# slinderman/pyglm

Hardware: AMD Instinct MI355X
Metric: Gibbs sweeps/sec (full resample_model) (higher is better)
Workload: dtype f64 (likelihood Gram: exact integer arithmetic on 13 i8 residue planes, CRT back to f64)

## Files before the change

### include/pyglm_hip.h

```cpp
#ifndef PYGLM_HIP_H
#define PYGLM_HIP_H
#include <stddef.h>
#include <stdint.h>
#ifdef __cplusplus
extern "C" {
#endif

#define PGL_ABI_VERSION 11

int pgl_abi_version(void);
const char* pgl_last_error(void);

int pgl_philox_words(uint64_t seed, uint32_t purpose, uint32_t j, uint64_t elem0, uint64_t stream, uint32_t* out, size_t n, void* hip_stream);

int pgl_pg_draw(const double* b, const double* z, double* out, size_t len, uint64_t seed, uint64_t stream, uint64_t elem0, void* hip_stream);

int pgl_design_matrix(const double* S, long lds, const double* basis, double* X, long ldx, double* Xt, long ldxt, int T, int N, int B, int R,
                      int clip, void* hip_stream);
int pgl_transpose(const double* src, long ld_src, double* dst, long ld_dst, int rows, int cols, void* hip_stream);

int pgl_activation(const double* Xt, long ldxt, const double* Wt, long ldw, double* Psi, long ldpsi, int T, int Dk, int nloc, void* hip_stream);

int pgl_pg_loglik(double* Psi, long ldpsi, const double* bias, const double* Y, long ldy, double* Omega, long ldo, double* Kappa, long ldk,
                  double* llpart, double* ll_out, int accumulate, int T, int nloc, int obs, double xi, uint64_t seed, uint64_t sweep,
// ... 111 lines not shown
    int obs; double xi;
    int visit_order;
    int planes, i8_group;
    const pgl_dataset_t* datasets; int ndatasets;
    int* a; double* W; double* b;
    const double* rho;
    const double* Jw; const double* hw; const int* label;
    const double* Jb; const double* hb;
    const double* c0;
    const int* perm; const double* u; const double* z;
    const double* inv_eta; const double* G0;
    double* ll;
    int* status;
    double* logodds;
    double* Wt; double* bias; double* border; int* skip; double* c0_dense;
    double* Jbuf; double* Mtab; double* Ac;
    double* hc; double* Tinv; double* G; double* Lws;
    double* Ut; double* Wt_ws;
    int* d_idx; double* d_sign; int* d_cnt; int* batch_k;
    int* act; int* na;
    void* i8_PB; void* i8_R; double* i8_stat;
    int i8_slice;
    void* i8_PAs;
    void* i8_Rx;
    double* i8_norm;
    int nrun;
    int nfirst;
    int all_deterministic;
    int init_rows_bound;
    int active_rows_bound;
    int flip_single_pass;
    pgl_stage_times_t* times;
    const double* obs_param;
} pgl_sweep_t;

int pgl_sweep_dims(int N, int B, int nloc, int* Dp, int* ldn, int* ldj);
int pgl_row_stats(const int* a, const double* W, double* out, int N, int B, int nloc, int n0, void* hip_stream);
int pgl_sweep(const pgl_sweep_t* s, uint64_t seed, uint64_t sweep, void* hip_stream);
int pgl_sweep_gram(const pgl_sweep_t* s, int first, int count, void* hip_stream);
int pgl_get_state(const pgl_sweep_t* s, int* a_host, double* W_host, double* b_host, double* ll_host, int* status_host, void* hip_stream);
const char* pgl_stage_name(int i);
int pgl_stage_times_collect(pgl_stage_times_t* t);

int pgl_summary_fold(const double* Psi, long ldn, const double* bias, const double* Y, double* llpart, double* ll_out, int accumulate, int T,
                     int nloc, int obs, double xi, const double* param, const double* hooks, long ldh, const double* inv_eta, double* rate_mean,
                     double* rate_M2, const int* link, int link0, const double* link_par, double link_par0, double* l_mean, double* l_M2,
                     double* lse_m, double* lse_s, int k, void* hip_stream);
int pgl_summary_state(const int* a, const double* Wt, long ldw, const double* bias, double* edge, double* w_mean, double* w_M2, double* b_mean,
                      double* b_M2, int N, int B, int nloc, int k, void* hip_stream);
int pgl_summary_colsum(const double* V, long ldv, int T, int nloc, double* part, double* out, int accumulate, void* hip_stream);

size_t pgl_generate_work_bytes(int N, int B);
int pgl_generate(const double* Wm, const double* bias, const double* basis, int N, int B, int L, int obs, double noise_scale, const double* U,
                 double* ring, double* Y, long t0, int Tc, void* work, int* status, void* hip_stream);

#define PGL_SIM_BINOMIAL_MAX_N 64
size_t pgl_simulate_work_bytes(int N, int B, int R);
int pgl_simulate(const double* Wm, const double* bias, const double* basis, int N, int B, int L, const int* kind, const double* par, int R,
                 long rep0, unsigned long long seed, double* ring, double* Y, long ldr, double* sum, double* sumsq, long t0, int Tc,
                 void* work, int* status, void* hip_stream);

#define PGL_LAG_MAX 256
#define PGL_LAG_I8 0
#define PGL_LAG_F64 1
size_t pgl_lagged_work_bytes(int N, int K, int R, int rows);
int pgl_lagged_products(const double* Y, long ldy, long strideY, int rows, int prev, int N, int K, int R, double* S, long strideS, int accumulate,
// ... 24 lines not shown
```

### pyglm_amd/_lib.py

```python
import ctypes
import os

_HERE = os.path.dirname(os.path.abspath(__file__))
LIB_PATH = os.path.join(_HERE, "lib", "libpyglm_hip.so")

c_p, c_l, c_i, c_d, c_u64, c_u32, c_sz = (ctypes.c_void_p, ctypes.c_long, ctypes.c_int, ctypes.c_double,
                                          ctypes.c_uint64, ctypes.c_uint32, ctypes.c_size_t)


class FlipState(ctypes.Structure):
    _fields_ = [("M", c_p), ("ldj", c_l), ("strideM", c_l), ("nb", c_i), ("N", c_i), ("B", c_i),
                ("perm", c_p), ("u", c_p), ("rho", c_p), ("c0", c_p), ("a", c_p), ("skip", c_p),
                ("d_idx", c_p), ("d_sign", c_p), ("d_cnt", c_p), ("batch_k", c_p), ("G", c_p), ("Lws", c_p),
                ("Ut", c_p), ("Wt", c_p), ("ldu", c_l), ("status", c_p), ("visit_order", c_i), ("logodds", c_p)]


class CholState(ctypes.Structure):
    _fields_ = [("J", c_p), ("ldj", c_l), ("strideJ", c_l), ("a", c_p), ("act", c_p), ("ldact", c_l), ("na", c_p),
                ("Ac", c_p), ("ldc", c_l), ("strideC", c_l), ("hc", c_p), ("Tinv", c_p), ("z", c_p), ("ldz", c_l),
                ("W", c_p), ("b", c_p), ("nb", c_i), ("N", c_i), ("B", c_i), ("status", c_p)]


class Dataset(ctypes.Structure):
    _fields_ = [("T", c_i), ("Tp", c_i), ("X", c_p), ("Xt", c_p), ("Y", c_p), ("Psi", c_p), ("OK", c_p), ("llpart", c_p), ("elem0", c_u64),
                ("int8", c_i), ("planes", c_i), ("sA", c_p), ("PA", c_p), ("omega_override", c_p), ("xmax", c_p),
                ("hooks", c_p)]


NSTAGES = 16


class StageTimes(ctypes.Structure):
    _fields_ = [("ms", c_d * NSTAGES), ("work", c_d * NSTAGES), ("calls", c_i * NSTAGES), ("pending", c_p), ("mask", c_u32)]


class Sweep(ctypes.Structure):
    _fields_ = [("N", c_i), ("B", c_i), ("n0", c_i), ("nloc", c_i), ("nb", c_i), ("obs", c_i), ("xi", c_d), ("visit_order", c_i),
                ("planes", c_i), ("i8_group", c_i), ("datasets", ctypes.POINTER(Dataset)), ("ndatasets", c_i),
                ("a", c_p), ("W", c_p), ("b", c_p), ("rho", c_p), ("Jw", c_p), ("hw", c_p), ("label", c_p), ("Jb", c_p), ("hb", c_p), ("c0", c_p),
                ("perm", c_p), ("u", c_p), ("z", c_p), ("inv_eta", c_p), ("G0", c_p), ("ll", c_p), ("status", c_p), ("logodds", c_p),
                ("Wt", c_p), ("bias", c_p), ("border", c_p), ("skip", c_p), ("c0_dense", c_p),
                ("Jbuf", c_p), ("Mtab", c_p), ("Ac", c_p), ("hc", c_p), ("Tinv", c_p), ("G", c_p), ("Lws", c_p), ("Ut", c_p), ("Wt_ws", c_p),
                ("d_idx", c_p), ("d_sign", c_p), ("d_cnt", c_p), ("batch_k", c_p), ("act", c_p), ("na", c_p),
                ("i8_PB", c_p), ("i8_R", c_p), ("i8_stat", c_p), ("i8_slice", c_i), ("i8_PAs", c_p), ("i8_Rx", c_p), ("i8_norm", c_p), ("nrun", c_i), ("nfirst", c_i),
                ("all_deterministic", c_i), ("init_rows_bound", c_i), ("active_rows_bound", c_i), ("flip_single_pass", c_i),
                ("times", ctypes.POINTER(StageTimes)), ("obs_param", c_p)]


SIGNATURES = {
    "pgl_abi_version": [],
    "pgl_last_error": [],
    "pgl_philox_words": [c_u64, c_u32, c_u32, c_u64, c_u64, c_p, c_sz, c_p],
    "pgl_pg_draw": [c_p, c_p, c_p, c_sz, c_u64, c_u64, c_u64, c_p],
    "pgl_design_matrix": [c_p, c_l, c_p, c_p, c_l, c_p, c_l, c_i, c_i, c_i, c_i, c_i, c_p],
    "pgl_transpose": [c_p, c_l, c_p, c_l, c_i, c_i, c_p],
    "pgl_activation": [c_p, c_l, c_p, c_l, c_p, c_l, c_i, c_i, c_i, c_p],
    "pgl_pg_loglik": [c_p, c_l, c_p, c_p, c_l, c_p, c_l, c_p, c_l, c_p, c_p, c_i, c_i, c_i, c_i, c_d, c_u64, c_u64, c_u64, c_u64, c_p],
    "pgl_pg_loglik_partials": [c_i],
    "pgl_pg_loglik_ex": [c_p, c_l, c_p, c_p, c_l, c_p, c_l, c_p, c_l, c_p, c_p, c_i, c_i, c_i, c_i, c_d, c_p, c_p, c_l, c_u64, c_u64, c_u64, c_u64, c_p],
    "pgl_gaussian_stats": [c_p, c_l, c_p, c_p, c_l, c_p, c_p, c_l, c_p, c_l, c_p, c_p, c_i, c_i, c_i, c_p],
    "pgl_scaled_gram": [c_p, c_l, c_p, c_p, c_l, c_l, c_i, c_i, c_p],
    "pgl_weighted_gram": [c_p, c_l, c_i, c_p, c_l, c_i, c_i, c_i, c_p, c_l, c_l, c_i, c_p],
    "pgl_i8_plane_bytes": [c_i, c_i],
    "pgl_i8_residue_bytes": [c_i],
    "pgl_i8_max_planes": [],
    "pgl_i8_padded_rows": [c_i],
    "pgl_i8_min_planes": [c_i],
    "pgl_i8_norm_bits": [c_i, c_i],
    "pgl_i8_norm_limit": [c_i, c_i],
    "pgl_i8_colstats": [c_p, c_l, c_p, c_l, c_i, c_i, c_i, c_p, c_p, c_p],
    "pgl_i8_scales": [c_p, c_p, c_l, c_i, c_i, c_p, c_p],
    "pgl_i8_planes": [c_p, c_l, c_p, c_l, c_p, c_p, c_i, c_i, c_i, c_i, c_l, c_p],
    "pgl_i8_planes_t": [c_p, c_l, c_p, c_l, c_p, c_p, c_i, c_i, c_i, c_i, c_l, c_p],
    "pgl_i8_gram": [c_p, c_p, c_p, c_i, c_i, c_i, c_i, c_p],
    "pgl_i8_gram_slice": [c_p, c_i, c_i, c_p, c_p, c_i, c_i, c_i, c_i, c_i, c_i, c_p],
    "pgl_i8_crt": [c_p, c_p, c_p, c_p, c_l, c_l, c_i, c_i, c_i, c_i, c_i, c_p],
    "pgl_contract_tn": [c_p, c_l, c_i, c_p, c_l, c_i, c_p, c_l, c_i, c_i, c_i, c_d, c_d, c_p],
    "pgl_contract_tn_batched": [c_p, c_l, c_l, c_i, c_p, c_l, c_l, c_i, c_p, c_l, c_l, c_i, c_i, c_i, c_i, c_p, c_d, c_d, c_i, c_i, c_p],
    "pgl_assemble_posterior": [c_p, c_l, c_l, c_p, c_p, c_l, c_p, c_p, c_p, c_p, c_p, c_i, c_i, c_i, c_p],
# ... 87 lines not shown
```

### pyglm_amd/csrc/pgl_common.h

```cpp
#pragma once
#include <hip/hip_runtime.h>
#include <stdint.h>
#include <stddef.h>
#include <atomic>
#include "../../include/pyglm_hip.h"

#define PGL_OK 0
#define PGL_ERR_ARG 1
#define PGL_ERR_HIP 2

void pgl_set_error(const char* fmt, ...);

#ifdef PGL_AB
#include <cstdlib>
inline int pgl_ab_int(const char* name, int dflt) { const char* e = getenv(name); return e ? atoi(e) : dflt; }
#else
constexpr int pgl_ab_int(const char*, int dflt) { return dflt; }
#endif

constexpr int PGL_MAX_DEVICES = 32;
int pgl_device();
int pgl_device_cus(int dev);
struct PglPerDevice {
    std::atomic<uint32_t> mask{0};
// ... 10 lines not shown
            pgl_set_error("%s:%d: argument check failed: %s", __FILE__, __LINE__, #cond); \
            return PGL_ERR_ARG;                                                          \
        }                                                                                \
    } while (0)

#define PGL_CHECK_LAUNCH()                                                                         \
    do {                                                                                           \
        hipError_t e_ = hipGetLastError();                                                         \
        if (e_ != hipSuccess) {                                                                    \
            pgl_set_error("%s:%d: kernel launch failed: %s", __FILE__, __LINE__, hipGetErrorString(e_)); \
            return PGL_ERR_HIP;                                                                    \
        }                                                                                          \
    } while (0)

typedef double d4_t __attribute__((ext_vector_type(4)));
typedef double d2_t __attribute__((ext_vector_type(2)));

struct PglGemmArgs {
    const double* A; long lda; long strideA;
    const double* B; long ldb; long strideB;
    double* C; long ldc; long strideC;
    const double* W; long ldw;
    int M, N, K;
    int a_cols, b_cols;
    int nbatch;
    int nz_total;
    double alpha, beta;
    int tri;
    const int* batch_k;
    int* sched;
    const int* batch_dim; int dim_off;
    int dim_mode;
    const int* batch_row_off;
    int pipe;
    int ksplit; long ks_rows; double* Cpart; long part_stride_z, part_stride_s;
};
enum PglGemmKind { PGL_GEMM_GRAM2 = 0, PGL_GEMM_PLAIN = 1, PGL_GEMM_TRI1 = 2, PGL_GEMM_SQUARES = 3 };
int pgl_launch_gemm(PglGemmKind kind, const PglGemmArgs& a, hipStream_t st);
int pgl_gram_split(const double* X, long ldx, int x_cols, const double* W, long ldw, int Tp, int D, int nz, double* J, long ldj, long strideJ, int accumulate,
                   long ks_rows, double* part, long part_stride_z, hipStream_t st);
bool pgl_update_supported(const PglGemmArgs& a);
int pgl_launch_update(const PglGemmArgs& a, hipStream_t st);
int pgl_launch_update_rows(const PglGemmArgs& a, int row0, int nrows, hipStream_t st);
int* pgl_sched_slot(hipStream_t st);

int pgl_k_philox_words(uint64_t, uint32_t, uint32_t, uint64_t, uint64_t, uint32_t*, size_t, hipStream_t);
int pgl_k_pg_draw(const double*, const double*, double*, size_t, uint64_t, uint64_t, uint64_t, hipStream_t);
int pgl_k_row_stats(const int* a, const double* W, double* out, int N, int B, int nloc, int n0, hipStream_t st);
int pgl_k_colsum_partials(const double* part, int nblk, int ncol, double* out, int accumulate, hipStream_t st);
int pgl_k_summary_state(const int* a, const double* Wt, long ldw, const double* bias, double* edge, double* wmean, double* wM2, double* bmean,
                        double* bM2, int N, int B, int nloc, int k, hipStream_t st);
int pgl_k_summary_colsum(const double* V, long ldv, int T, int nloc, double* part, double* out, int accumulate, hipStream_t st);
int pgl_k_scaled_gram(const double*, long, const double*, double*, long, long, int, int, hipStream_t);
int pgl_k_basis_conv(const double*, long, const double*, double*, long, double*, long, int, int, int, int, int, hipStream_t);
int pgl_k_transpose(const double*, long, double*, long, int, int, hipStream_t);
int pgl_k_assemble_post(double*, long, long, const double*, const double*, long, const double*, const double*, const int*, const double*,
                        const double*, int, int, int, hipStream_t);
size_t pgl_k_i8_plane_bytes(int, int);
size_t pgl_k_i8_residue_bytes(int);
int pgl_k_i8_max_planes(void);
int pgl_k_i8_padded_rows(int);
int pgl_k_i8_min_planes(int);
int pgl_k_i8_nu(int, int);
double pgl_k_i8_norm_limit(int, int);
int pgl_k_i8_colstats(const double*, long, const double*, long, int, int, int, double*, double*, hipStream_t);
int pgl_k_i8_scales(const double*, const double*, long, int, int, double*, hipStream_t);
int pgl_k_i8_colmax(const double*, long, int, int, double*, hipStream_t);
int pgl_k_i8_scales_bound(const double*, long, const double*, const double*, int, int, int, int, double*, hipStream_t);
int pgl_k_i8_colstats_scales(const double*, long, const double*, long, int, int, int, int, double*, double*, hipStream_t);
int pgl_k_i8_planes(const double*, long, int transposed, const double*, long, const double*, int8_t*, int, int, int, int, long t_base, hipStream_t);
int pgl_k_i8_gram(const int8_t*, long, int, const int8_t*, int8_t*, int8_t*, int, int, int, int, int, hipStream_t);
long pgl_k_i8_kp(int);
int pgl_k_i8_crt(const int8_t*, const int8_t*, const double*, const double*, double*, long, long, int, int, int, int, hipStream_t);
int pgl_k_flip_apply(const pgl_flip_t&, int, int, int, hipStream_t);
int pgl_k_flip_apply_pair(const pgl_flip_t&, int phase, int window, int* ws, hipStream_t);
int pgl_k_flip_permute(const pgl_flip_t&, const double*, long, long, hipStream_t);
int pgl_k_flip_decide(const pgl_flip_t&, int, hipStream_t);
int pgl_k_flip_pivot_list(const pgl_flip_t&, int*, long, int*, hipStream_t);
int pgl_k_flip_pivot_chunk(const pgl_flip_t&, const int*, long, const int*, int, int, hipStream_t);
int pgl_k_flip_kmax(void);
int pgl_k_flip_window_blocks(int);
int pgl_k_chol_index(const pgl_chol_t&, hipStream_t);
bool pgl_k_small_fits(int N, int B);
int pgl_k_small_max_rows(void);
int pgl_k_small_tail(const double* J, long ldj, long strideJ, int nb, int N, int B, const int* perm, const double* u, const double* rho, const double* c0,
                     int* a, const int* skip, const double* z, long ldz, double* W, double* b, int* status, double* logodds, hipStream_t st);
int pgl_k_chol_sample(const pgl_chol_t&, int, hipStream_t);
```

### pyglm_amd/csrc/pgl_flips.hip

```cpp
#include "pgl_common.h"

namespace {

constexpr int KMAX = 512;
constexpr int KWIN = 320;

struct FlipArgs {
    double* M; long ldj; long strideM;
    int N, B, R;
    const int* perm;
    const double* u;
    const double* rho;
    const double* c0;
    int* a;
    const int* skip;
    int* d_idx;
    double* d_sign;
    int* d_cnt;
    int* batch_k;
    double* G;
    double* Lws;
    double* Ut; double* Wt; long ldu;
    int* status;
    int permuted;
// ... 686 lines not shown
    w.A = s.G; w.lda = KMAX; w.strideA = (long)KMAX * KMAX;
    w.B = s.Ut + r0; w.ldb = s.ldu; w.strideB = (long)KMAX * s.ldu;
    w.C = s.Wt + r0; w.ldc = s.ldu; w.strideC = (long)KMAX * s.ldu;
    w.M = KMAX; w.N = ncol; w.K = KMAX; w.a_cols = KMAX; w.b_cols = ncol; w.nbatch = s.nb; w.nz_total = 0;
    w.alpha = 1.0; w.beta = 0.0; w.tri = 0; w.batch_k = s.batch_k; w.batch_dim = s.batch_k; w.dim_off = 0; w.dim_mode = 2; w.W = nullptr; w.ldw = 0;
    w.pipe = 1;
    int rc = pgl_launch_gemm(PGL_GEMM_PLAIN, w, st);
    if (rc) return rc;
    static const bool patch_ab = pgl_ab_int("PGL_FLIP_PATCH", 0) != 0;
    const bool patch = r0 == 0 && patch_ab;
    if (patch) {
        hipLaunchKernelGGL(patch_pivot_cols_kernel, dim3(64, s.nb), dim3(256), 0, st, g);
        PGL_CHECK_LAUNCH();
    }
    PglGemmArgs t{};
    t.A = s.Wt + r0; t.lda = s.ldu; t.strideA = (long)KMAX * s.ldu;
    t.B = s.Ut + r0; t.ldb = s.ldu; t.strideB = (long)KMAX * s.ldu;
    t.C = s.M + (long)r0 * s.ldj + r0; t.ldc = s.ldj; t.strideC = s.strideM;
    t.M = Md - r0; t.N = Md - r0; t.K = KMAX; t.a_cols = ncol; t.b_cols = ncol; t.nbatch = s.nb; t.nz_total = 0;
    t.alpha = -1.0; t.beta = 1.0; t.tri = 1; t.batch_k = s.batch_k; t.batch_dim = nullptr; t.dim_off = 0; t.W = nullptr; t.ldw = 0;
    t.pipe = 1;
    rc = pgl_launch_gemm(PGL_GEMM_TRI1, t, st);
    if (rc) return rc;
    if (patch) {
        hipLaunchKernelGGL(diag_fix_kernel, dim3(KMAX / 256, s.nb), dim3(256), 0, st, g);
        PGL_CHECK_LAUNCH();
    } else if (r0 == 0) {
        hipLaunchKernelGGL(fixup_kernel, dim3((Md + GT - 1) / GT, KMAX / GT, s.nb), dim3(256), 0, st, g);
        PGL_CHECK_LAUNCH();
    }
    return PGL_OK;
}

__global__ __launch_bounds__(256) void pair_plan_first_kernel(const int* __restrict__ batch_k, int nb, int room, int* __restrict__ ws) {
    const int n = blockIdx.x * 256 + threadIdx.x;
    if (n >= nb) return;
    const int k1 = batch_k[n];
    const bool paired = k1 + room <= KMAX;
    ws[n] = paired ? k1 : 0;
    ws[nb + n] = paired ? 0 : k1;
    ws[2 * nb + n] = paired ? k1 : 0;
}
__global__ __launch_bounds__(256) void pair_plan_second_kernel(const int* __restrict__ batch_k, int nb, int* __restrict__ ws) {
    const int n = blockIdx.x * 256 + threadIdx.x;
    if (n < nb) ws[3 * nb + n] = ws[n] + batch_k[n];
}

int pgl_k_flip_apply_pair(const pgl_flip_t& s, int phase, int window, int* ws, hipStream_t st) {
    const int R_ = pgl_k_flip_window_blocks(s.B);
    const int Md = s.N * s.B + 2;
    if (!s.visit_order || (long)(window + 1) * R_ >= s.N) return PGL_OK;
    const int r0 = ((window + 1) * R_ * s.B) & ~1;
    FlipArgs g = mk(s, R_, r0, phase ? ws : nullptr);
    hipLaunchKernelGGL(gather_panel_kernel, dim3((unsigned)((s.ldu - r0 + GT - 1) / GT), KMAX / GT, s.nb), dim3(256), 0, st, g);
    PGL_CHECK_LAUNCH();
    const int ncol = (int)s.ldu - r0;
    PglGemmArgs w{};
    w.A = s.G; w.lda = KMAX; w.strideA = (long)KMAX * KMAX;
    w.B = s.Ut + r0; w.ldb = s.ldu; w.strideB = (long)KMAX * s.ldu;
    w.C = s.Wt + r0; w.ldc = s.ldu; w.strideC = (long)KMAX * s.ldu;
    w.M = KMAX; w.N = ncol; w.K = KMAX; w.a_cols = KMAX; w.b_cols = ncol; w.nbatch = s.nb;
    w.alpha = 1.0; w.beta = 0.0; w.tri = 0; w.batch_k = s.batch_k; w.batch_dim = s.batch_k; w.dim_off = 0; w.dim_mode = 2;
    w.batch_row_off = phase ? ws : nullptr;
    w.pipe = 1;
    if (int rc = pgl_launch_gemm(PGL_GEMM_PLAIN, w, st)) return rc;
    PglGemmArgs t{};
    t.A = s.Wt + r0; t.lda = s.ldu; t.strideA = (long)KMAX * s.ldu;
    t.B = s.Ut + r0; t.ldb = s.ldu; t.strideB = (long)KMAX * s.ldu;
    t.C = s.M + (long)r0 * s.ldj + r0; t.ldc = s.ldj; t.strideC = s.strideM;
    t.M = Md - r0; t.N = Md - r0; t.K = KMAX; t.a_cols = ncol; t.b_cols = ncol; t.nbatch = s.nb;
    t.alpha = -1.0; t.beta = 1.0; t.tri = 1; t.pipe = 1;
    if (phase == 0) {
        const int room = (R_ * s.B + 15) & ~15;
        hipLaunchKernelGGL(pair_plan_first_kernel, dim3((s.nb + 255) / 256), dim3(256), 0, st, s.batch_k, s.nb, room, ws);
        PGL_CHECK_LAUNCH();
        t.batch_k = ws + s.nb;
        if (int rc = pgl_launch_gemm(PGL_GEMM_TRI1, t, st)) return rc;
        const int nblk1 = min(R_, s.N - (window + 1) * R_);
        PglGemmArgs q = t;
        q.N = (window + 1) * R_ * s.B + nblk1 * s.B - r0; q.tri = 0; q.pipe = 0; q.batch_k = ws + 2 * s.nb;
        return pgl_launch_gemm(PGL_GEMM_PLAIN, q, st);
    }
    hipLaunchKernelGGL(pair_plan_second_kernel, dim3((s.nb + 255) / 256), dim3(256), 0, st, s.batch_k, s.nb, ws);
    PGL_CHECK_LAUNCH();
    t.batch_k = ws + 3 * s.nb;
    return pgl_launch_gemm(PGL_GEMM_TRI1, t, st);
}

int pgl_k_flip_permute(const pgl_flip_t& s, const double* J, long ldjs, long strideJ, hipStream_t st) {
    FlipArgs g = mk(s, 0);
    g.permuted = 1;
    const dim3 grid(1, s.N + 2, s.nb);
#define PGL_PERMUTE(b_) case b_: hipLaunchKernelGGL(permute_tableau_kernel<b_>, grid, dim3(256), 0, st, g, J, ldjs, strideJ); break;
    switch (s.B) {
        PGL_PERMUTE(1) PGL_PERMUTE(2) PGL_PERMUTE(3) PGL_PERMUTE(4) PGL_PERMUTE(5) PGL_PERMUTE(6) PGL_PERMUTE(7) PGL_PERMUTE(8)
        default: hipLaunchKernelGGL(permute_tableau_kernel<0>, grid, dim3(256), 0, st, g, J, ldjs, strideJ); break;
    }
#undef PGL_PERMUTE
    PGL_CHECK_LAUNCH();
    return PGL_OK;
}

int pgl_k_flip_decide(const pgl_flip_t& s, int window, hipStream_t st) {
    const int R = pgl_k_flip_window_blocks(s.B);
    if (R < 1) { pgl_set_error("B=%d exceeds the window capacity %d", s.B, KWIN); return PGL_ERR_ARG; }
    FlipArgs g = mk(s, R);
    const size_t lds = pgl_k_flip_lds_decide(s.B, R);
#define PGL_DECIDE(b_)                                                                                                      \
    case b_: {                                                                                                              \
        static PglPerDeviceSize lds_set_b;                                                                                  \
        if (int rc = pgl_grow_dynamic_lds(reinterpret_cast<const void*>(decide_kernel<b_>), lds, lds_set_b)) return rc;     \
        hipLaunchKernelGGL(decide_kernel<b_>, dim3(s.nb), dim3(1024), lds, st, g, window);                                  \
    } break;
    switch (s.B <= 8 ? s.B : 0) {
        PGL_DECIDE(0) PGL_DECIDE(1) PGL_DECIDE(2) PGL_DECIDE(3) PGL_DECIDE(4) PGL_DECIDE(5) PGL_DECIDE(6) PGL_DECIDE(7) PGL_DECIDE(8)
        default: break;
    }
#undef PGL_DECIDE
    PGL_CHECK_LAUNCH();
// ... 20 lines not shown
```

### pyglm_amd/csrc/pgl_gemm.hip

```cpp
#include "pgl_common.h"
#include <type_traits>

namespace {

constexpr int BK = 16;
constexpr int PAD = 16;

template <int WM, int WN, int WZ, bool WEIGHTED, int STAGES = 2>
struct Cfg {
    static constexpr int BM = WM * 64, BN = WN * 64;
    static constexpr int SA = BM + PAD, SB = BN + PAD;
    static constexpr int THREADS = WM * WN * WZ * 64;
    static constexpr int A_ELEMS = BK * SA, B_ELEMS = BK * SB, W_ELEMS = WEIGHTED ? BK * WZ : 0;
    static constexpr int STAGE = A_ELEMS + B_ELEMS + W_ELEMS;
    static constexpr size_t LDS_BYTES = (size_t)STAGES * STAGE * sizeof(double);
    static constexpr int A_LD = (BK * BM / 2) / THREADS, B_LD = (BK * BN / 2) / THREADS;
    static_assert((BK * BM / 2) % THREADS == 0 && (BK * BN / 2) % THREADS == 0, "tile/threads mismatch");
};

__device__ __forceinline__ int isqrt_tri(int t) {
    int r = (int)((__builtin_sqrt(8.0 * (double)t + 1.0) - 1.0) * 0.5);
    while ((long)(r + 1) * (r + 2) / 2 <= t) ++r;
    while ((long)r * (r + 1) / 2 > t) --r;
    return r;
// ... 11 lines not shown
    const int ntm = (g.M + C::BM - 1) / C::BM;
    int tile, batch, tm, tn;
    if (g.nbatch > 1) {
        if (WEIGHTED || (g.strideA == 0 && g.strideB == 0)) {
            tile = (int)(w / g.nbatch); batch = (int)(w % g.nbatch);
        } else {
            const int ntn_ = (g.N + C::BN - 1) / C::BN;
            const long ntiles = g.tri ? (long)ntm * (ntm + 1) / 2 : (long)ntm * ntn_;
            batch = (int)(w / ntiles); tile = (int)(w % ntiles);
        }
    } else { tile = (int)w; batch = 0; }
    if (g.tri) { tm = isqrt_tri(tile); tn = tile - tm * (tm + 1) / 2; if (g.tri == 2) { const int s_ = tm; tm = tn; tn = s_; } }
    else { tm = tile % ntm; tn = tile / ntm; }
    int Mv = g.M, Nv = g.N;
    if (g.batch_dim) {
        const int d = g.batch_dim[batch] - g.dim_off;
        if (g.dim_mode == 0) { Mv = d; Nv = d; }
        else if (g.dim_mode == 1) Nv = d;
        else if (g.dim_mode == 2) Mv = d;
        else { Mv = g.M < d ? g.M : d; Nv = d; }
    }
    if (tm * C::BM >= Mv || tn * C::BN >= Nv) return;

    int K = g.K;
    if (g.batch_k) { K = g.batch_k[batch]; if (K <= 0) return; }
    const int nkt = K / BK;

    const int tid = threadIdx.x, lane = tid & 63, wave = tid >> 6;
    const int wz = wave / (WM * WN), wmn = wave % (WM * WN), wm = wmn / WN, wn = wmn % WN;
    const int m0 = tm * C::BM, n0 = tn * C::BN;

    const double* __restrict__ Ab = g.A + (long)batch * g.strideA;
    const long roff_ = g.batch_row_off ? (long)g.batch_row_off[batch] : 0;
    const double* __restrict__ Bb = g.B + (long)batch * g.strideB + roff_ * g.ldb;
    const int zg = batch * WZ + wz;
    const bool zvalid = !WEIGHTED || zg < g.nz_total;

    d2_t ra[C::A_LD], rb[C::B_LD];
    double rw = 0.0;
    const unsigned long long aflip = (CINIT && g.alpha < 0.0) ? 0x8000000000000000ull : 0ull;
    typedef unsigned long long u2_t __attribute__((ext_vector_type(2)));
    auto signed_a = [&](d2_t v) { return __builtin_bit_cast(d2_t, __builtin_bit_cast(u2_t, v) ^ u2_t{aflip, aflip}); };
    unsigned oa_[C::A_LD], ob_[C::B_LD], ow_ = 0;
    const char* ka_ = reinterpret_cast<const char*>(Ab);
    const char* kb_ = reinterpret_cast<const char*>(Bb);
    const char* kw_ = reinterpret_cast<const char*>(g.W);
#pragma unroll
    for (int i = 0; i < C::A_LD; ++i) {
        const int p = tid + i * C::THREADS, r = p / (C::BM / 2), c = (p % (C::BM / 2)) * 2;
        int col = m0 + c;
        col = col < g.a_cols ? col : g.a_cols - 2;
        oa_[i] = (unsigned)(((long)r * g.lda + col) * 8);
    }
#pragma unroll
    for (int i = 0; i < C::B_LD; ++i) {
        const int p = tid + i * C::THREADS, r = p / (C::BN / 2), c = (p % (C::BN / 2)) * 2;
        int col = n0 + c;
        col = col < g.b_cols ? col : g.b_cols - 2;
        ob_[i] = (unsigned)(((long)r * g.ldb + col) * 8);
    }
    if (WEIGHTED) {
        const int t_ = tid < BK * WZ ? tid : 0, r = t_ / WZ, z = t_ % WZ;
        int zc = batch * WZ + z;
        zc = zc < g.nz_total ? zc : g.nz_total - 1;
        ow_ = (unsigned)(((long)r * g.ldw + zc) * 8);
    }
    const long stepA = (long)BK * g.lda * 8, stepB = (long)BK * g.ldb * 8, stepW = (long)BK * g.ldw * 8;
// ... 732 lines not shown
```

### pyglm_amd/csrc/pgl_sweep.hip

```cpp
#include "pgl_common.h"
#include "pgl_obs.h"
#include <cmath>
#include <tuple>
#include <vector>

namespace {

__global__ __launch_bounds__(256) void pack_weights_kernel(const int* __restrict__ a, const double* __restrict__ W, const double* __restrict__ b,
                                                           double* __restrict__ Wt, double* __restrict__ bias, int N, int B, int nloc, int Dp, int ldn) {
    const long e = (long)blockIdx.x * 256 + threadIdx.x;
    if (e < nloc) bias[e] = b[e];
    if (e >= (long)Dp * ldn) return;
    const int d = (int)(e / ldn), n = (int)(e % ldn), D = N * B;
    double v = 0.0;
    if (d < D && n < nloc && a[(long)n * N + d / B]) v = W[(long)n * D + d];
    Wt[e] = v;
}

__global__ __launch_bounds__(256) void deterministic_rows_kernel(const double* __restrict__ rho, int* __restrict__ a, int* __restrict__ skip, int N) {
    const int n = blockIdx.x;
    __shared__ int s_any;
    if (threadIdx.x == 0) s_any = 0;
    __syncthreads();
    int bad = 0;
// ... 335 lines not shown
        }
        if (s->visit_order && pgl_k_small_fits(N, B)) {
            auto ms = clk.tic(ST_FLIPS);
            RC(pgl_k_small_tail(s->Jbuf, ldj, strideJ, nbb, N, B, s->perm + (long)s0 * N, s->u + (long)s0 * N, s->rho + (long)s0 * N, c0 + (long)s0 * N,
                                s->a + (long)s0 * N, s->skip + s0, s->z + (long)s0 * (D + 1), D + 1, s->W + (long)s0 * D, s->b + s0, s->status + s0,
                                s->logodds ? s->logodds + (long)s0 * N : nullptr, st));
            clk.toc(ms);
            continue;
        }
        auto mf = clk.tic(ST_FLIPS);
        if (!s->all_deterministic) {
            pgl_flip_t fs{};
            fs.M = s->Mtab; fs.ldj = ldj; fs.strideM = strideJ; fs.nb = nbb; fs.N = N; fs.B = B;
            fs.perm = s->perm + (long)s0 * N; fs.u = s->u + (long)s0 * N; fs.rho = s->rho + (long)s0 * N; fs.c0 = c0 + (long)s0 * N;
            fs.a = s->a + (long)s0 * N; fs.skip = s->skip + s0;
            fs.d_idx = s->d_idx; fs.d_sign = s->d_sign; fs.d_cnt = s->d_cnt; fs.batch_k = s->batch_k;
            fs.G = s->G; fs.Lws = s->Lws; fs.Ut = s->Ut; fs.Wt = s->Wt_ws; fs.ldu = ldj;
            fs.status = s->status + s0; fs.visit_order = s->visit_order ? 1 : 0; fs.logodds = s->logodds ? s->logodds + (long)s0 * N : nullptr;
            if (s->visit_order) RC(pgl_k_flip_permute(fs, s->Jbuf, ldj, strideJ, st));
            else if (hipMemcpyAsync(s->Mtab, s->Jbuf, (size_t)nbb * strideJ * sizeof(double), hipMemcpyDeviceToDevice, st) != hipSuccess) {
                pgl_set_error("tableau copy failed"); return PGL_ERR_HIP;
            }
            RC(pgl_k_flip_pivot_list(fs, s->act, D + 1, s->na, st));
            const int ck = kmax;
            long rows = s->init_rows_bound > 0 && s->init_rows_bound <= D + 1 ? s->init_rows_bound : D + 1;
            for (int c = 0; (long)c * ck < rows; ++c) {
                const long left = (D + 1) - (long)c * ck;
                auto m = clk.tic(ST_FINIT);
                RC(pgl_k_flip_pivot_chunk(fs, s->act, D + 1, s->na, c, ck, st));
                RC(pgl_k_flip_apply(fs, 0, (int)(left < ck ? left : ck), -1, st));
                clk.toc(m);
            }
            const int nwin = (N + R - 1) / R;
            const bool pair = s->visit_order && !s->flip_single_pass;
            for (int w = 0; w < nwin; ++w) {
                auto m = clk.tic(ST_FDEC);
                RC(pgl_k_flip_decide(fs, w, st));
                clk.toc(m);
                m = clk.tic(ST_FAPP);
                if (!pair || (w % 2 == 0 && w + 1 >= nwin)) RC(pgl_k_flip_apply(fs, 1, 0, w, st));
                else RC(pgl_k_flip_apply_pair(fs, w % 2, w, s->act, st));
                clk.toc(m);
            }
        }
        clk.toc(mf);
        auto mw = clk.tic(ST_W);
        pgl_chol_t cs{};
        cs.J = s->Jbuf; cs.ldj = ldj; cs.strideJ = strideJ; cs.a = s->a + (long)s0 * N;
        cs.act = s->act; cs.ldact = D + 1; cs.na = s->na;
        cs.Ac = s->Ac; cs.ldc = ldj; cs.strideC = strideJ; cs.hc = s->hc; cs.Tinv = s->Tinv;
        cs.z = s->z + (long)s0 * (D + 1); cs.ldz = D + 1; cs.W = s->W + (long)s0 * D; cs.b = s->b + s0;
        cs.nb = nbb; cs.N = N; cs.B = B; cs.status = s->status + s0;
        RC(pgl_k_chol_index(cs, st));
        long na_bound = s->active_rows_bound > 0 && s->active_rows_bound <= D + 1 ? s->active_rows_bound : D + 1;
        RC(pgl_k_chol_sample(cs, (int)na_bound, st));
        clk.toc(mw);
    }
    return PGL_OK;
}

int pgl_sweep_gram(const pgl_sweep_t* s, int first, int count, void* hip_stream) {
    RC(check_gram_args(s));
    PGL_CHECK_ARG(first >= 0 && count > 0 && count <= s->nb && first + count <= s->nloc);
    hipStream_t st = reinterpret_cast<hipStream_t>(hip_stream);
    Clock clk{s->times, st};
    return gram_batch(*s, first, count, clk, st);
}

int pgl_get_state(const pgl_sweep_t* s, int* a_host, double* W_host, double* b_host, double* ll_host, int* status_host, void* hip_stream) {
    hipStream_t st = reinterpret_cast<hipStream_t>(hip_stream);
    PGL_CHECK_ARG(s && s->nloc > 0);
    const long D = (long)s->N * s->B;
    auto cp = [&](void* dst, const void* src, size_t bytes) { return dst == nullptr || hipMemcpyAsync(dst, src, bytes, hipMemcpyDeviceToHost, st) == hipSuccess; };
    bool ok = cp(a_host, s->a, (size_t)s->nloc * s->N * sizeof(int)) && cp(W_host, s->W, (size_t)s->nloc * D * sizeof(double)) &&
// ... 8 lines not shown
```

### pyglm_amd/csrc/pgl_update.hip

```cpp
#include "pgl_common.h"

namespace {

constexpr int BK = 16;
constexpr int PAD = 16;
constexpr int NST = 3;
constexpr int SBMAJ = 4, SBMIN = 8;

template <bool WIDE_B>
struct UCfg {
    static constexpr int BM = WIDE_B ? 128 : 256, BN = WIDE_B ? 256 : 128;
    static constexpr int SA = BM + PAD, SB = BN + PAD;
    static constexpr int A_ELEMS = BK * SA, B_ELEMS = BK * SB, STAGE = A_ELEMS + B_ELEMS;
    static constexpr size_t LDS_BYTES = (size_t)NST * STAGE * sizeof(double) + 32;
};

struct UpdArgs {
    PglGemmArgs g;
    int nmaj, nmin;
    int ntiles;
    int cinit;
    int stagger;
};

// ... 373 lines not shown
            u.g.sched = nullptr;
            hipLaunchKernelGGL(update_rows_kernel, dim3((unsigned)((a0.N + 127) / 128), (unsigned)a0.nbatch), dim3(256), 0, st, u, row0, extra);
            PGL_CHECK_LAUNCH();
            u.g.M = row0; u.g.N = row0;
        }
    }
    const PglGemmArgs& a = u.g;
    const int ntm = (a.M + C::BM - 1) / C::BM, ntn = (a.N + C::BN - 1) / C::BN;
    u.nmaj = WIDE_B ? ntn : ntm;
    u.nmin = WIDE_B ? ntm : ntn;
    long nt = 0;
    for (int m = 0; m < u.nmaj; ++m) {
        int hi = u.nmin - 1;
        if (a.tri && 2 * m + 1 < hi) hi = 2 * m + 1;
        nt += hi + 1;
    }
    u.ntiles = (int)nt;
    u.stagger = u.cinit;
    const long total = nt * a.nbatch;
    if (total <= 0) return PGL_OK;
    if (total > 0x7fffffffL) { pgl_set_error("update: %ld work items", total); return PGL_ERR_ARG; }
    u.g.sched = pgl_sched_slot(st);
    if (!u.g.sched) { pgl_set_error("update: scheduler scratch unavailable"); return PGL_ERR_HIP; }
    const int n_cu = pgl_device_cus(pgl_device());
    const long grid = total < n_cu ? total : n_cu;
    hipLaunchKernelGGL(kern, dim3((unsigned)grid), dim3(512), C::LDS_BYTES, st, u);
    PGL_CHECK_LAUNCH();
    return PGL_OK;
}

}

bool pgl_update_supported(const PglGemmArgs& a) {
    if (a.W != nullptr || a.K % BK != 0 || a.M <= 0 || a.N <= 0 || a.nbatch <= 0) return false;
    if (!((a.beta == 1.0 && (a.alpha == 1.0 || a.alpha == -1.0)) || a.beta == 0.0)) return false;
    if (a.tri != 0 && a.M != a.N) return false;
    if (a.a_cols % 2 || a.b_cols % 2 || a.lda % 2 || a.ldb % 2 || a.a_cols < 2 || a.b_cols < 2) return false;
    if (((uintptr_t)a.A % 16) || ((uintptr_t)a.B % 16) || (a.strideA % 2) || (a.strideB % 2)) return false;
    return true;
}

int pgl_launch_update(const PglGemmArgs& a, hipStream_t st) {
    if (!pgl_update_supported(a)) { pgl_set_error("update pipeline: unsupported product"); return PGL_ERR_ARG; }
    return a.tri == 2 ? launch_update<true>(a, st) : launch_update<false>(a, st);
}

int pgl_launch_update_rows(const PglGemmArgs& a, int row0, int nrows, hipStream_t st) {
    if (!pgl_update_supported(a) || nrows < 1 || nrows > 16 || row0 < 0 || a.batch_dim != nullptr) { pgl_set_error("update rows: unsupported product"); return PGL_ERR_ARG; }
    UpdArgs u{};
    u.g = a;
    u.cinit = a.beta == 1.0 ? 1 : 0;
    hipLaunchKernelGGL(update_rows_kernel, dim3((unsigned)((a.N + 127) / 128), (unsigned)a.nbatch), dim3(256), 0, st, u, row0, nrows);
    PGL_CHECK_LAUNCH();
    return PGL_OK;
}
```

### pyglm_amd/engine.py

```python
import ctypes
import functools
import time
import typing

import numpy as np
import torch

from . import _lib
from ._lib import call, ptr

F64 = torch.float64
I32 = torch.int32


def _r(x, m):
    return (x + m - 1) // m * m


def _on_device(fn):
    @functools.wraps(fn)
    def wrapped(self, *args, **kwargs):
        with torch.cuda.device(self.dev):
            return fn(self, *args, **kwargs)
    return wrapped
# ... 87 lines not shown
            self._i8_over = dict(group=i8_group, slice=i8_slice, resident=i8_resident)
            self._device_share = max(1, int(device_share))
            self._init(N, B, obs, xi, batch, mem_budget_bytes, design_only, visit_order, gram, likelihood_only, planes)

    def _init(self, N, B, obs, xi, batch, mem_budget_bytes, design_only, visit_order, gram, likelihood_only, planes):
        self.obs = self.OBS[obs]
        self.xi, self.obs_param = self._obs_param(xi)
        self.Dp = _r(self.D + 1, 16)
        self.ldn = _r(self.nloc, 2)
        self.ldj = _r(self.D + 2, 16)
        self.kmax = _lib.load().pgl_flip_kmax()
        self.R = _lib.load().pgl_flip_window_blocks(self.B)
        if self.R < 1:
            raise ValueError("B=%d too large for the proposal window" % self.B)
        self.datasets = []
        self.gram = gram or "auto"
        assert self.gram in ("auto", "fp64", "int8")
        self.planes = int(planes) if planes else None
        assert self.planes is None or 1 <= self.planes <= _lib.load().pgl_i8_max_planes()
        self._i8_scratch = None
        self.visit_order = bool(visit_order)
        self.share_tableau = self.visit_order
        self._batch_arg, self._mem_budget = batch, mem_budget_bytes
        self.nb = None
        self.design_only = design_only
        self.likelihood_only = bool(likelihood_only)
        if likelihood_only:
            self._alloc_shard()
        elif not design_only:
            self._alloc_shard()
            if batch is not None:
                self._ensure_batch()
        self.flip_single_pass = False
        self.keep_logodds = False
        self.logodds = None
        self.profile = False
        self._times = None
        self._i8_norm = None
        self._ev = []
        self.wait_seconds = 0.0
        self.overlap_seconds = 0.0
        self.launch_seconds = 0.0

    def _obs_param(self, xi):
        v = np.asarray(xi, dtype=np.float64)
        if v.ndim == 0:
            vals, out = v.reshape(1), (float(v), None)
        else:
            v = v.reshape(-1)
            if v.size == self.N:
                v = v[self.n0:self.n1]
            elif v.size != self.nloc:
                raise ValueError("xi: %d values for a model of %d neurons (shard of %d)" % (v.size, self.N, self.nloc))
            vals, out = v, (1.0, torch.from_numpy(np.ascontiguousarray(v)).to(self.dev))
        if self.obs == 1 and not np.all(vals > 0):
            raise ValueError("negative binomial: xi must be > 0")
        if self.obs == 3 and not np.all((vals >= 0) & (vals == np.floor(vals))):
            raise ValueError("binomial: the number of trials n must be an integer >= 0")
        return out

    def _tic(self, name, work=0.0):
        if not self.profile:
            return None
        e0 = torch.cuda.Event(enable_timing=True)
        e1 = torch.cuda.Event(enable_timing=True)
        e0.record(torch.cuda.current_stream(self.dev))
# ... 561 lines not shown
        if isinstance(Jw, BlockPrior):
            label, c0, hw, Jw = Jw.label, Jw.c0_u, Jw.hw_u, Jw.Jw_u
        off_a, off_W, off_b, off_ll, off_st, sb = self._io_state_layout()
        items = [("rho", rho, np.float64), ("Jw", Jw, np.float64), ("hw", hw, np.float64), ("Jb", Jb, np.float64), ("hb", hb, np.float64),
                 ("c0", c0, np.float64), ("perm", perm, np.int32), ("u", u, np.float64), ("z", z, np.float64)]
        if label is not None:
            items.append(("label", label, np.int32))
        arrs, offs, off = {}, {}, sb
        for k, v, dt in items:
            arr = np.ascontiguousarray(v, dtype=dt)
            arrs[k], offs[k] = arr, off
            off = (off + arr.nbytes + 15) // 16 * 16
        self._io_reserve(off - sb)
        hin = self._hin_np
        hin[off_a:off_a + 4 * nloc * N].view(np.int32)[:] = a.reshape(-1)
        hin[off_W:off_W + 8 * nloc * D].view(np.float64)[:] = np.asarray(W, dtype=np.float64).reshape(-1)
        hin[off_b:off_b + 8 * nloc].view(np.float64)[:] = np.asarray(b, dtype=np.float64).reshape(-1)
        for k, arr in arrs.items():
            hin[offs[k]:offs[k] + arr.nbytes] = arr.reshape(-1).view(np.uint8)
        self._din[:off].copy_(self._hin[:off], non_blocking=True)
        base = self._din.data_ptr()
        dp = {k: ctypes.c_void_p(base + o) for k, o in offs.items()}
        dp.setdefault("label", None)
        self.logodds = torch.empty((nloc, N), dtype=F64, device=self.dev) if self.keep_logodds else None
        if label is not None and (self._c0_dense is None):
            self._c0_dense = self._z(nloc, N)
        ovs = None
        if omega_override is not None:
            ovs = [torch.from_numpy(np.ascontiguousarray(omega_override[i], dtype=np.float64).reshape(ds.T, nloc)).to(self.dev)
                   for i, ds in enumerate(self.datasets)]
        sw = self._sweep_args(ovs)
        sw.rho, sw.Jw, sw.hw, sw.label, sw.Jb, sw.hb, sw.c0 = dp["rho"], dp["Jw"], dp["hw"], dp["label"], dp["Jb"], dp["hb"], dp["c0"]
        sw.perm, sw.u, sw.z = dp["perm"], dp["u"], dp["z"]
        sw.logodds, sw.c0_dense = ptr(self.logodds), ptr(self._c0_dense)
        n_act = int(a.sum(axis=1).max()) if a.size else 0
        sw.nrun, sw.nfirst, sw.all_deterministic = int(nrun), int(nfirst), int(det.all())
        sw.init_rows_bound = 1 + B * n_act
        sw.active_rows_bound = (1 + B * int(np.round(rho).sum(axis=1).max())) if det.all() else 0
        sw.flip_single_pass = int(self.flip_single_pass)
        t_launch = time.perf_counter()
        call("pgl_sweep", ctypes.byref(sw), int(seed), int(sweep), st)
        self.launch_seconds += time.perf_counter() - t_launch
        self.last_row_stats = None
        if want_stats:
            if getattr(self, "_stats_dev", None) is None:
                self._stats_dev = torch.empty((nloc, 1 + B + B * B), dtype=F64, device=self.dev)
                self._stats_host = torch.empty((nloc, 1 + B + B * B), dtype=F64).pin_memory()
            call("pgl_row_stats", ptr(self.a_dev), ptr(self.W_dev), ptr(self._stats_dev), N, B, nloc, self.n0, st)
            self._stats_host.copy_(self._stats_dev, non_blocking=True)
        if after_queue is not None:
            after_queue(self)
        if host_overlap is not None:
            t_ov = time.perf_counter()
            host_overlap()
            self.overlap_seconds += time.perf_counter() - t_ov
        t_wait = time.perf_counter()
        hout = self._hout_np
        hp = self._hout.data_ptr()
        call("pgl_get_state", ctypes.byref(sw), ctypes.c_void_p(hp + off_a) if readback else None, ctypes.c_void_p(hp + off_W) if readback else None,
             ctypes.c_void_p(hp + off_b) if readback else None, ctypes.c_void_p(hp + off_ll), ctypes.c_void_p(hp + off_st), st)
        self.wait_seconds += time.perf_counter() - t_wait
        a_i = hout[off_a:off_a + 4 * nloc * N].view(np.int32).reshape(nloc, N) if readback else None
        W_new = hout[off_W:off_W + 8 * nloc * D].view(np.float64).reshape(nloc, N, B) if readback else None
        b_new = hout[off_b:off_b + 8 * nloc].view(np.float64) if readback else None
        if readback and copy:
            W_new, b_new = W_new.copy(), b_new.copy()
        ll = hout[off_ll:off_ll + 8 * nloc].view(np.float64).copy()
# ... 50 lines not shown
```

Measured before the change: 0.05826.

## Generalize paired flip window updates to stacked multi-window deferred updates

Replaces the two-window pairing scheme for applying flip rank updates with a stacking scheme. Deferred update columns accumulate across as many consecutive windows as fit in KMAX. Each window first corrects its panel against the stacked prior updates with a small GEMM, and only the near-diagonal block is updated eagerly. This cuts the number of full trailing rank-K updates of the tableau, at the cost of extra gathers, a stack-correction GEMM, and more complex bookkeeping. An optional debug buffer records the maximum stack depth.

```diff
diff --git a/include/pyglm_hip.h b/include/pyglm_hip.h
--- a/include/pyglm_hip.h
+++ b/include/pyglm_hip.h
@@ -167,6 +167,7 @@
     int flip_single_pass;
     pgl_stage_times_t* times;
     const double* obs_param;
+    int* flip_stack_depth;
 } pgl_sweep_t;
 
 int pgl_sweep_dims(int N, int B, int nloc, int* Dp, int* ldn, int* ldj);
diff --git a/pyglm_amd/_lib.py b/pyglm_amd/_lib.py
--- a/pyglm_amd/_lib.py
+++ b/pyglm_amd/_lib.py
@@ -44,7 +44,7 @@
                 ("d_idx", c_p), ("d_sign", c_p), ("d_cnt", c_p), ("batch_k", c_p), ("act", c_p), ("na", c_p),
                 ("i8_PB", c_p), ("i8_R", c_p), ("i8_stat", c_p), ("i8_slice", c_i), ("i8_PAs", c_p), ("i8_Rx", c_p), ("i8_norm", c_p), ("nrun", c_i), ("nfirst", c_i),
                 ("all_deterministic", c_i), ("init_rows_bound", c_i), ("active_rows_bound", c_i), ("flip_single_pass", c_i),
-                ("times", ctypes.POINTER(StageTimes)), ("obs_param", c_p)]
+                ("times", ctypes.POINTER(StageTimes)), ("obs_param", c_p), ("flip_stack_depth", c_p)]
 
 
 SIGNATURES = {
diff --git a/pyglm_amd/csrc/pgl_common.h b/pyglm_amd/csrc/pgl_common.h
--- a/pyglm_amd/csrc/pgl_common.h
+++ b/pyglm_amd/csrc/pgl_common.h
@@ -66,6 +66,7 @@
     const int* batch_dim; int dim_off;
     int dim_mode;
     const int* batch_row_off;
+    int row_off_c_only;
     int pipe;
     int ksplit; long ks_rows; double* Cpart; long part_stride_z, part_stride_s;
 };
@@ -107,7 +108,7 @@
 long pgl_k_i8_kp(int);
 int pgl_k_i8_crt(const int8_t*, const int8_t*, const double*, const double*, double*, long, long, int, int, int, int, hipStream_t);
 int pgl_k_flip_apply(const pgl_flip_t&, int, int, int, hipStream_t);
-int pgl_k_flip_apply_pair(const pgl_flip_t&, int phase, int window, int* ws, hipStream_t);
+int pgl_k_flip_apply_stack(const pgl_flip_t&, int window, int* ws, int* depth_max, hipStream_t);
 int pgl_k_flip_permute(const pgl_flip_t&, const double*, long, long, hipStream_t);
 int pgl_k_flip_decide(const pgl_flip_t&, int, hipStream_t);
 int pgl_k_flip_pivot_list(const pgl_flip_t&, int*, long, int*, hipStream_t);
diff --git a/pyglm_amd/csrc/pgl_flips.hip b/pyglm_amd/csrc/pgl_flips.hip
--- a/pyglm_amd/csrc/pgl_flips.hip
+++ b/pyglm_amd/csrc/pgl_flips.hip
@@ -742,59 +742,80 @@
     return PGL_OK;
 }
 
-__global__ __launch_bounds__(256) void pair_plan_first_kernel(const int* __restrict__ batch_k, int nb, int room, int* __restrict__ ws) {
+__global__ __launch_bounds__(256) void stack_cols_kernel(FlipArgs g, const int* __restrict__ off, int room) {
+    const int n = blockIdx.y, K = off[n], cnt = g.d_cnt[n], kp = (cnt + 15) & ~15;
+    if (K <= 0 || cnt <= 0) return;
+    const int* idx = g.d_idx + (long)n * KMAX;
+    const double* Ut = g.Ut + (long)n * KMAX * g.ldu;
+    double* Uc = g.G + (long)n * KMAX * KMAX + (long)room * KMAX;
+    for (int e = blockIdx.x * 256 + threadIdx.x; e < K * kp; e += gridDim.x * 256) {
+        const int k = e / kp, q = e - k * kp;
+        Uc[(long)k * KMAX + q] = q < cnt ? Ut[(long)k * g.ldu + idx[q]] : 0.0;
+    }
+}
+__global__ __launch_bounds__(256) void stack_plan_kernel(const int* __restrict__ batch_k, int nb, int room, int* __restrict__ ws, int* __restrict__ depth_max) {
     const int n = blockIdx.x * 256 + threadIdx.x;
     if (n >= nb) return;
-    const int k1 = batch_k[n];
-    const bool paired = k1 + room <= KMAX;
-    ws[n] = paired ? k1 : 0;
-    ws[nb + n] = paired ? 0 : k1;
-    ws[2 * nb + n] = paired ? k1 : 0;
-}
-__global__ __launch_bounds__(256) void pair_plan_second_kernel(const int* __restrict__ batch_k, int nb, int* __restrict__ ws) {
-    const int n = blockIdx.x * 256 + threadIdx.x;
-    if (n < nb) ws[3 * nb + n] = ws[n] + batch_k[n];
-}
-
-int pgl_k_flip_apply_pair(const pgl_flip_t& s, int phase, int window, int* ws, hipStream_t st) {
+    const int k = batch_k[n], off = ws[n] + k;
+    const int depth = ws[3 * nb + n] + (k > 0);
+    const bool stack = off + room <= KMAX;
+    ws[n] = stack ? off : 0;
+    ws[nb + n] = stack ? 0 : off;
+    ws[2 * nb + n] = stack ? off : 0;
+    ws[3 * nb + n] = stack ? depth : 0;
+    if (depth_max && depth > depth_max[n]) depth_max[n] = depth;
+}
+
+int pgl_k_flip_apply_stack(const pgl_flip_t& s, int window, int* ws, int* depth_max, hipStream_t st) {
     const int R_ = pgl_k_flip_window_blocks(s.B);
-    const int Md = s.N * s.B + 2;
+    const int D = s.N * s.B, Md = D + 2;
     if (!s.visit_order || (long)(window + 1) * R_ >= s.N) return PGL_OK;
+    if (window == 0 && hipMemsetAsync(ws, 0, (size_t)4 * s.nb * sizeof(int), st) != hipSuccess) { pgl_set_error("memset failed"); return PGL_ERR_HIP; }
     const int r0 = ((window + 1) * R_ * s.B) & ~1;
-    FlipArgs g = mk(s, R_, r0, phase ? ws : nullptr);
+    const int rl = (D + 1) & ~1;
+    const int room = (R_ * s.B + 15) & ~15;
+    const int ncol = (int)s.ldu - r0;
+    FlipArgs g = mk(s, R_, r0, ws);
     hipLaunchKernelGGL(gather_panel_kernel, dim3((unsigned)((s.ldu - r0 + GT - 1) / GT), KMAX / GT, s.nb), dim3(256), 0, st, g);
     PGL_CHECK_LAUNCH();
-    const int ncol = (int)s.ldu - r0;
+    if (window > 0 && room < KMAX) {
+        hipLaunchKernelGGL(stack_cols_kernel, dim3(16, s.nb), dim3(256), 0, st, g, (const int*)ws, room);
+        PGL_CHECK_LAUNCH();
+        PglGemmArgs c{};
+        c.A = s.G + (long)room * KMAX; c.lda = KMAX; c.strideA = (long)KMAX * KMAX;
+        c.B = s.Wt + r0; c.ldb = s.ldu; c.strideB = (long)KMAX * s.ldu;
+        c.C = s.Ut + r0; c.ldc = s.ldu; c.strideC = (long)KMAX * s.ldu;
+        c.M = room; c.N = rl - r0; c.K = KMAX; c.a_cols = KMAX; c.b_cols = ncol; c.nbatch = s.nb;
+        c.alpha = -1.0; c.beta = 1.0; c.tri = 0; c.batch_k = ws; c.batch_dim = s.d_cnt; c.dim_off = 0; c.dim_mode = 2;
+        c.batch_row_off = ws; c.row_off_c_only = 1;
+        if (int rc = pgl_launch_gemm(PGL_GEMM_PLAIN, c, st)) return rc;
+    }
     PglGemmArgs w{};
     w.A = s.G; w.lda = KMAX; w.strideA = (long)KMAX * KMAX;
     w.B = s.Ut + r0; w.ldb = s.ldu; w.strideB = (long)KMAX * s.ldu;
     w.C = s.Wt + r0; w.ldc = s.ldu; w.strideC = (long)KMAX * s.ldu;
     w.M = KMAX; w.N = ncol; w.K = KMAX; w.a_cols = KMAX; w.b_cols = ncol; w.nbatch = s.nb;
     w.alpha = 1.0; w.beta = 0.0; w.tri = 0; w.batch_k = s.batch_k; w.batch_dim = s.batch_k; w.dim_off = 0; w.dim_mode = 2;
-    w.batch_row_off = phase ? ws : nullptr;
+    w.batch_row_off = ws;
     w.pipe = 1;
     if (int rc = pgl_launch_gemm(PGL_GEMM_PLAIN, w, st)) return rc;
+    hipLaunchKernelGGL(stack_plan_kernel, dim3((s.nb + 255) / 256), dim3(256), 0, st, s.batch_k, s.nb, room, ws, depth_max);
+    PGL_CHECK_LAUNCH();
     PglGemmArgs t{};
     t.A = s.Wt + r0; t.lda = s.ldu; t.strideA = (long)KMAX * s.ldu;
     t.B = s.Ut + r0; t.ldb = s.ldu; t.strideB = (long)KMAX * s.ldu;
     t.C = s.M + (long)r0 * s.ldj + r0; t.ldc = s.ldj; t.strideC = s.strideM;
     t.M = Md - r0; t.N = Md - r0; t.K = KMAX; t.a_cols = ncol; t.b_cols = ncol; t.nbatch = s.nb;
     t.alpha = -1.0; t.beta = 1.0; t.tri = 1; t.pipe = 1;
-    if (phase == 0) {
-        const int room = (R_ * s.B + 15) & ~15;
-        hipLaunchKernelGGL(pair_plan_first_kernel, dim3((s.nb + 255) / 256), dim3(256), 0, st, s.batch_k, s.nb, room, ws);
-        PGL_CHECK_LAUNCH();
-        t.batch_k = ws + s.nb;
-        if (int rc = pgl_launch_gemm(PGL_GEMM_TRI1, t, st)) return rc;
-        const int nblk1 = min(R_, s.N - (window + 1) * R_);
-        PglGemmArgs q = t;
-        q.N = (window + 1) * R_ * s.B + nblk1 * s.B - r0; q.tri = 0; q.pipe = 0; q.batch_k = ws + 2 * s.nb;
-        return pgl_launch_gemm(PGL_GEMM_PLAIN, q, st);
-    }
-    hipLaunchKernelGGL(pair_plan_second_kernel, dim3((s.nb + 255) / 256), dim3(256), 0, st, s.batch_k, s.nb, ws);
-    PGL_CHECK_LAUNCH();
-    t.batch_k = ws + 3 * s.nb;
-    return pgl_launch_gemm(PGL_GEMM_TRI1, t, st);
+    t.batch_k = ws + s.nb;
+    if (int rc = pgl_launch_gemm(PGL_GEMM_TRI1, t, st)) return rc;
+    const int nblk1 = min(R_, s.N - (window + 1) * R_);
+    PglGemmArgs q = t;
+    q.M = q.N = (window + 1) * R_ * s.B + nblk1 * s.B - r0; q.tri = 0; q.pipe = 0; q.batch_k = ws + 2 * s.nb;
+    if (int rc = pgl_launch_gemm(PGL_GEMM_PLAIN, q, st)) return rc;
+    PglGemmArgs h = q;
+    h.A = s.Wt + rl; h.a_cols = (int)s.ldu - rl; h.C = s.M + (long)rl * s.ldj + r0; h.M = Md - rl;
+    return pgl_launch_gemm(PGL_GEMM_PLAIN, h, st);
 }
 
 int pgl_k_flip_permute(const pgl_flip_t& s, const double* J, long ldjs, long strideJ, hipStream_t st) {
diff --git a/pyglm_amd/csrc/pgl_gemm.hip b/pyglm_amd/csrc/pgl_gemm.hip
--- a/pyglm_amd/csrc/pgl_gemm.hip
+++ b/pyglm_amd/csrc/pgl_gemm.hip
@@ -67,7 +67,7 @@
 
     const double* __restrict__ Ab = g.A + (long)batch * g.strideA;
     const long roff_ = g.batch_row_off ? (long)g.batch_row_off[batch] : 0;
-    const double* __restrict__ Bb = g.B + (long)batch * g.strideB + roff_ * g.ldb;
+    const double* __restrict__ Bb = g.B + (long)batch * g.strideB + (g.row_off_c_only ? 0 : roff_ * g.ldb);
     const int zg = batch * WZ + wz;
     const bool zvalid = !WEIGHTED || zg < g.nz_total;
 
diff --git a/pyglm_amd/csrc/pgl_sweep.hip b/pyglm_amd/csrc/pgl_sweep.hip
--- a/pyglm_amd/csrc/pgl_sweep.hip
+++ b/pyglm_amd/csrc/pgl_sweep.hip
@@ -391,14 +391,14 @@
                 clk.toc(m);
             }
             const int nwin = (N + R - 1) / R;
-            const bool pair = s->visit_order && !s->flip_single_pass;
+            const bool stack = s->visit_order && !s->flip_single_pass;
             for (int w = 0; w < nwin; ++w) {
                 auto m = clk.tic(ST_FDEC);
                 RC(pgl_k_flip_decide(fs, w, st));
                 clk.toc(m);
                 m = clk.tic(ST_FAPP);
-                if (!pair || (w % 2 == 0 && w + 1 >= nwin)) RC(pgl_k_flip_apply(fs, 1, 0, w, st));
-                else RC(pgl_k_flip_apply_pair(fs, w % 2, w, s->act, st));
+                if (!stack) RC(pgl_k_flip_apply(fs, 1, 0, w, st));
+                else RC(pgl_k_flip_apply_stack(fs, w, s->act, s->flip_stack_depth ? s->flip_stack_depth + s0 : nullptr, st));
                 clk.toc(m);
             }
         }
diff --git a/pyglm_amd/csrc/pgl_update.hip b/pyglm_amd/csrc/pgl_update.hip
--- a/pyglm_amd/csrc/pgl_update.hip
+++ b/pyglm_amd/csrc/pgl_update.hip
@@ -429,7 +429,7 @@
 }
 
 bool pgl_update_supported(const PglGemmArgs& a) {
-    if (a.W != nullptr || a.K % BK != 0 || a.M <= 0 || a.N <= 0 || a.nbatch <= 0) return false;
+    if (a.W != nullptr || a.K % BK != 0 || a.M <= 0 || a.N <= 0 || a.nbatch <= 0 || a.row_off_c_only) return false;
     if (!((a.beta == 1.0 && (a.alpha == 1.0 || a.alpha == -1.0)) || a.beta == 0.0)) return false;
     if (a.tri != 0 && a.M != a.N) return false;
     if (a.a_cols % 2 || a.b_cols % 2 || a.lda % 2 || a.ldb % 2 || a.a_cols < 2 || a.b_cols < 2) return false;
diff --git a/pyglm_amd/engine.py b/pyglm_amd/engine.py
--- a/pyglm_amd/engine.py
+++ b/pyglm_amd/engine.py
@@ -143,6 +143,8 @@
             if batch is not None:
                 self._ensure_batch()
         self.flip_single_pass = False
+        self.keep_flip_stack_depth = False
+        self.flip_stack_depth = None
         self.keep_logodds = False
         self.logodds = None
         self.profile = False
@@ -770,7 +772,8 @@
         sw = self._sweep_args(ovs)
         sw.rho, sw.Jw, sw.hw, sw.label, sw.Jb, sw.hb, sw.c0 = dp["rho"], dp["Jw"], dp["hw"], dp["label"], dp["Jb"], dp["hb"], dp["c0"]
         sw.perm, sw.u, sw.z = dp["perm"], dp["u"], dp["z"]
-        sw.logodds, sw.c0_dense = ptr(self.logodds), ptr(self._c0_dense)
+        self.flip_stack_depth = torch.zeros(nloc, dtype=I32, device=self.dev) if self.keep_flip_stack_depth else None
+        sw.logodds, sw.c0_dense, sw.flip_stack_depth = ptr(self.logodds), ptr(self._c0_dense), ptr(self.flip_stack_depth)
         n_act = int(a.sum(axis=1).max()) if a.size else 0
         sw.nrun, sw.nfirst, sw.all_deterministic = int(nrun), int(nfirst), int(det.all())
         sw.init_rows_bound = 1 + B * n_act
```

New measurement: 0.05847 (median of 6 runs). About the same (+0.4%).
